# AFIDclan/cuda-raytracing

Hardware: AMD Instinct MI355X
Metric: Mrays/sec + ms/frame, 70k-tri OBJ at 1920x1080 1spp; 1/2/4/8 MI355X (higher is better)
Workload: dtype f32

## Files before the change

cuda-raytracing_amd/csrc/rt_device_types.h:

```cpp
#pragma once
#include <cstdint>
#include "rt_math.h"

namespace rt {

constexpr int32_t kLeafFlag = (int32_t)0x80000000u;
constexpr int kSlotBits = 26;
constexpr int32_t kSlotMask = (1 << kSlotBits) - 1;
constexpr int kMaxStack = 64;
constexpr int32_t kBoxUnordered = 1;

RT_HD bool boxes_ordered(const float* w)
{
    return w[0] <= w[3] && w[1] <= w[4] && w[2] <= w[5] && w[6] <= w[9] && w[7] <= w[10] && w[8] <= w[11];
}


struct DevInstance {
    Q4 q_rot;
    Q4 q_pose;
    Q4 q_inv_pose;
    Q4 q_inv_rot;
    float pose_xyz[3];
    float inv_pose_xyz[3];
    float scale[3];
    float inv_scale[3];
    int32_t root_ref;
    int32_t material_index;
    int32_t mesh_index;
    int32_t exact_uv;
    int32_t identity_inv;
    int32_t unit_inv;
    int32_t pad_[2];
};

struct DevMaterial {
    float albedo[3];
    int32_t texture_width;
    int32_t texture_height;
    uint32_t texture_pitch;
    const uint8_t* texture;
    float roughness, metallic;
};

constexpr int kExMaxGroup = 32;
constexpr int kExPlanesA = 5, kExPlanesS = 7;

constexpr int kMaxViewInstances = 8;
constexpr int kMaxBatch = 32;

struct FrameParams {
    float kinv[9];
    float D[4];
    float origin[3];
    Q4 q_cam;
    uint8_t* img;
    int32_t rank, local_rows;
};

struct RenderParams {
    int32_t width, height;
    int32_t num_frames;
    FrameParams frames[kMaxBatch];
    const float4* records;
    const float* tri_uv;
    const int32_t* tri_id;
    const int32_t* leaf_count;
    const int32_t* mesh_flags;
    const DevInstance* instances;
    const DevMaterial* materials;
    int32_t num_instances;
    int32_t stack_depth;
    uint64_t pitch;
    int32_t local_rows, stripe_rows, rank, num_ranks;
    int32_t tiles_x, tiles_y;
    unsigned long long* trace;
    const int32_t* tile_order;
    int32_t* tile_cost;
    int32_t spp, bounces, lighting;
    int32_t sample_base;
    float4* ex_samples;
// ... 29 lines not shown
```

cuda-raytracing_amd/csrc/rt_kernels.hip:

```cpp
#include <hip/hip_runtime.h>
#include <algorithm>
#include <cstddef>
#include <cstdio>
#include <cstdlib>
#include <cstring>
#include <mutex>
#include <new>
#include <type_traits>
#include <vector>

#include "../../include/rt_hip.h"
#include "rt_device_types.h"
#include "rt_math.h"
#include "rt_scene_internal.h"

using namespace rt;



namespace {

constexpr int kBlock = 256;
constexpr int kTile = 16;
constexpr int kPrimBlock = 64;
// ... 77 lines not shown
    lds_int* lds;
    int* spill;
    int lds_depth;
    int sp;
    __device__ __forceinline__ void push(int32_t v)
    {
        if constexpr (SPILL) { if (sp < lds_depth) lds[sp * STRIDE] = v; else spill[sp - lds_depth] = v; }
        else lds[sp * STRIDE] = v;
        sp++;
    }
    __device__ __forceinline__ int32_t pop()
    {
        --sp;
        if constexpr (!SPILL) return lds[sp * STRIDE];
        int32_t v = lds[(sp < lds_depth ? sp : lds_depth - 1) * STRIDE];
        if (sp >= lds_depth) v = spill[sp - lds_depth];
        return v;
    }
};

typedef StackT<kBlock> Stack;

struct MeshRay {
    V3 ro, rd, dinv;
};

__device__ __forceinline__ MeshRay to_mesh_space(const DevInstance& in, V3 org, V3 dir)
{
    MeshRay r;
    r.rd = apply_quat(in.q_rot, dir);
    r.rd.x *= in.inv_scale[0]; r.rd.y *= in.inv_scale[1]; r.rd.z *= in.inv_scale[2];
    r.ro = apply_quat(in.q_pose, v3(org.x - in.pose_xyz[0], org.y - in.pose_xyz[1], org.z - in.pose_xyz[2]));
    r.ro.x *= in.inv_scale[0]; r.ro.y *= in.inv_scale[1]; r.ro.z *= in.inv_scale[2];
    r.dinv = v3(1.0f / r.rd.x, 1.0f / r.rd.y, 1.0f / r.rd.z);
    return r;
}

template <bool DEBUG, class STK, int OCT = -1, bool NEED_POP = false, class W>
__device__ __forceinline__ bool interior_apply_words(const W& w, const MeshRay& r, float hit_min,
                                                     int32_t& cur, STK& stack, Counters<DEBUG>& cnt)
{
    int32_t ra = __float_as_int(w[12]), rb = __float_as_int(w[13]);
    if constexpr (DEBUG) cnt.aabb += 2;
    float da, db;
    if constexpr (OCT < 0) {
        da = slab(w[0], w[1], w[2], w[3], w[4], w[5], r.dinv);
        db = slab(w[6], w[7], w[8], w[9], w[10], w[11], r.dinv);
    } else {
        da = slab_oct<OCT>(w[0], w[1], w[2], w[3], w[4], w[5], r.dinv);
        db = slab_oct<OCT>(w[6], w[7], w[8], w[9], w[10], w[11], r.dinv);
    }
    const bool a_near = da < db;
    const bool pa = da < hit_min, pb = db < hit_min;
    int32_t next = pa ? ra : rb;
    if (pa && pb) {
        stack.push(a_near ? rb : ra);
        next = a_near ? ra : rb;
        if constexpr (STK::kOptimistic) next = stack.sp > stack.lds_depth ? kSentinel : next;
    }
    cur = NEED_POP ? ((pa | pb) ? next : kNeedPop) : next;
    return pa || pb;
}

template <bool DEBUG, class STK, int OCT = -1, bool NEED_POP = false>
__device__ __forceinline__ bool interior_apply(float4 q0, float4 q1, float4 q2, float4 q3, const MeshRay& r, float hit_min,
                                               int32_t& cur, STK& stack, Counters<DEBUG>& cnt)
// ... 23 lines not shown
    V3 pt = r.ro + tt * r.rd;
    ok = ok && !(pt.x == FLT_MAX);
    V3 e0 = v3(t1.z, t1.w, t2.x), e1 = v3(t2.y, t2.z, t2.w);
    V3 e2 = pt - v0;
    float dot02 = dot(e0, e2), dot12 = dot(e1, e2);
    float u = (t3.z * dot02 - t3.y * dot12) * t3.w;
    float v = (t3.x * dot12 - t3.y * dot02) * t3.w;
    ok = ok && (u >= 0.0f) && (v >= 0.0f) && (u + v <= 1.0f);
    c.u = u; c.v = v;
    if (exact_uv) {
        c.uv = make_float2(0.0f, 0.0f);
        if (ok) {
            const float* q = p.tri_uv + (size_t)slot * 6;
            float w = 1.0f - u - v;
            c.uv.x = (w * q[0] + v * q[2]) + u * q[4];
            c.uv.y = (w * q[1] + v * q[3]) + u * q[5];
            ok = c.uv.x != FLT_MAX;
        }
    }
    bool accept = false;
    if (ok) {
        if constexpr (DEBUG) cnt.inside++;
        V3 loc = pt;
        if (EX || !identity_inv) {
            loc = v3(pt.x * in.scale[0], pt.y * in.scale[1], pt.z * in.scale[2]);
            loc = apply_quat(in.q_inv_pose, v3(loc.x - in.inv_pose_xyz[0], loc.y - in.inv_pose_xyz[1], loc.z - in.inv_pose_xyz[2]));
        }
        c.dist = magnitude(loc - org);
        if constexpr (EX) c.loc = loc;
        accept = (denom < 0) & ((hit_min == FLT_MAX) | (c.dist < hit_min));
    }
    return accept;
}

template <bool DEBUG, bool PROF, bool EX, bool COUNT, class STK, bool POPS, int OCT, bool ANYHIT = false, bool VIEW = false>
__device__ __forceinline__ void trace_loop(const RenderParams& p, const DevInstance& in, int inst_index, const MeshRay& r,
                                           V3 org, STK& stack, Hit& hit, Counters<DEBUG>& cnt, int* iters, int* pops, uint32_t vdelta = 0,
                                           float tmax = FLT_MAX)
{
    static_assert(!VIEW || (!DEBUG && !PROF && !EX), "view records: the timed primary kernels only");
    stack.sp = 0;
    stack.push(kSentinel);
    int32_t cur = in.root_ref;
    bool have = true;
    constexpr bool kNeedPopValue = !EX;
    int rem = -1;
    unsigned long long c_pop = 0, c_mem = 0, c_int = 0, c_leaf = 0, n_it = 0, n_int = 0, n_leaf = 0, t0 = 0, t1 = 0, t2 = 0, t3 = 0;
    unsigned long long n_g1 = 0, n_g2 = 0, n_g34 = 0;
    const bool exact_uv = in.exact_uv != 0, identity_inv = in.identity_inv != 0;
    do {
        if constexpr (PROF) t1 = __builtin_amdgcn_s_memtime();
        if constexpr (COUNT) (*iters)++;
        const bool interior = cur >= 0;
        if constexpr (DEBUG) cnt.pops += (interior || rem < 0) ? 1 : 0;
        if constexpr (POPS) *pops += (interior || rem < 0) ? 1 : 0;
        float4 r0, r1, r2, r3;
        const int32_t cur0 = __builtin_amdgcn_readfirstlane(cur);
        typedef float f16v __attribute__((ext_vector_type(16)));
        if constexpr (VIEW) {
            const bool one_entry = __ballot(cur != cur0) == 0ull;
            if (one_entry && cur0 >= 0) {
                f16v w;
                const uint32_t off = ((uint32_t)cur0 << 6) + vdelta;
                asm volatile("s_load_dwordx16 %0, %1, %2\n\ts_waitcnt lgkmcnt(0)" : "=s"(w) : "s"(p.records), "s"(off));
                have = interior_apply_words<DEBUG, STK, OCT, kNeedPopValue>(w, r, hit.min, cur, stack, cnt);
                if (kNeedPopValue ? cur == kNeedPop : !have) cur = stack.pop();
// ... 79 lines not shown
        }
        if (any_accept != 0ull) {
            hit.min = accept ? c.dist : hit.min;
            hit.slot = accept ? slot : hit.slot;
            hit.instance = accept ? inst_index : hit.instance;
            hit.u = accept ? (exact_uv ? c.uv.x : c.u) : hit.u;
            hit.v = accept ? (exact_uv ? c.uv.y : c.v) : hit.v;
            if constexpr (EX) { hit.loc.x = accept ? c.loc.x : hit.loc.x; hit.loc.y = accept ? c.loc.y : hit.loc.y; hit.loc.z = accept ? c.loc.z : hit.loc.z; }
            if constexpr (ANYHIT) {
                const bool done = accept & (c.dist < tmax);
                if constexpr (kNeedPopValue) cur = done ? kSentinel : cur;
                else {
                    have = done ? false : have;
                    rem = done ? -1 : rem;
                    stack.sp = done ? 1 : stack.sp;
                }
            }
        }
        if constexpr (PROF) { __builtin_amdgcn_s_waitcnt(0); t0 = __builtin_amdgcn_s_memtime(); }
        if (kNeedPopValue ? cur == kNeedPop : !have) cur = stack.pop();
        __builtin_amdgcn_wave_barrier();
        if constexpr (PROF) {
            __builtin_amdgcn_s_waitcnt(0);
            c_mem += t2 - t1; c_int += t3 - t2; c_leaf += t0 - t3; c_pop += __builtin_amdgcn_s_memtime() - t0;
        }
    } while (cur != kSentinel);
    if constexpr (PROF) {
        if (p.trace) {
            unsigned long long v[10] = {c_pop, c_mem, c_int, c_leaf, n_it, n_int, n_leaf, n_g1, n_g2, n_g34};
            unsigned long long best = n_it;
            for (int o = 32; o > 0; o >>= 1) { unsigned long long x = __shfl_xor(best, o); best = x > best ? x : best; }
            const unsigned long long owner = __ballot(n_it == best);
            if ((int)(threadIdx.x & 63) == __ffsll((long long)owner) - 1) {
                unsigned long long* t = p.trace + (((size_t)blockIdx.y * gridDim.x + blockIdx.x) * (kPrimBlock / 64) + (threadIdx.x >> 6)) * 16 + 4;
                for (int k = 0; k < 10; k++) t[k] += v[k];
            }
        }
    }
}


#define RT_ASM_INTERIOR(AXN, AXF, AYN, AYF, AZN, AZF, BXN, BXF, BYN, BYF, BZN, BZF) \
    "v_mul_f32 v16, " AXN ", %[dix]\n\t"  "v_mul_f32 v17, " AYN ", %[diy]\n\t"  "v_mul_f32 v18, " AZN ", %[diz]\n\t" \
    "v_mul_f32 v19, " AXF ", %[dix]\n\t"  "v_mul_f32 v20, " AYF ", %[diy]\n\t"  "v_mul_f32 v21, " AZF ", %[diz]\n\t" \
    "v_max3_f32 v16, v16, v17, v18\n\t"                  \
    "v_min3_f32 v19, v19, v20, v21\n\t"                  \
    "v_mul_f32 v22, " BXN ", %[dix]\n\t"  "v_mul_f32 v23, " BYN ", %[diy]\n\t"  "v_mul_f32 v24, " BZN ", %[diz]\n\t" \
    "v_mul_f32 v25, " BXF ", %[dix]\n\t"  "v_mul_f32 v26, " BYF ", %[diy]\n\t"  "v_mul_f32 v27, " BZF ", %[diz]\n\t" \
    "v_max3_f32 v22, v22, v23, v24\n\t"                  \
    "v_min3_f32 v25, v25, v26, v27\n\t"                  \
    "v_cmp_ge_f32_e32 vcc, v19, v16\n\t" \
    "v_cmp_lt_f32_e64 s[38:39], 0, v19\n\t" \
    "v_cmp_lt_f32_e64 s[44:45], v16, %[hmin]\n\t" \
    "v_cmp_ge_f32_e64 s[40:41], v25, v22\n\t" \
    "v_cmp_lt_f32_e64 s[42:43], 0, v25\n\t" \
    "v_cmp_lt_f32_e64 s[66:67], v22, %[hmin]\n\t" \
    "v_cmp_lt_f32_e64 s[68:69], v16, v22\n\t"            \
    "s_and_b64 vcc, vcc, s[38:39]\n\t" \
    "s_and_b64 s[40:41], s[40:41], s[42:43]\n\t" \
    "s_and_b64 s[38:39], vcc, s[44:45]\n\t"              \
    "s_and_b64 s[40:41], s[40:41], s[66:67]\n\t"         \
    "s_orn2_b64 s[42:43], s[68:69], s[40:41]\n\t" \
    "s_and_b64 s[44:45], s[38:39], s[40:41]\n\t"         \
    "s_and_b64 s[42:43], s[42:43], s[38:39]\n\t"         \
    "s_or_b64 vcc, s[38:39], s[40:41]\n\t"               \
    "v_cndmask_b32_e64 v18, v13, v12, s[42:43]\n\t" \
    "s_and_saveexec_b64 s[38:39], s[44:45]\n\t" \
// ... 395 lines not shown
#undef RT_ASM_ORG_C
#undef RT_ASM_CASE_ANYHIT
    } else {
#define RT_ASM_ORG_C "s"
#define RT_ASM_CASE_ANYHIT(VN, SN)
        RT_ASM_ALL_CASES
#undef RT_ASM_ORG_C
#undef RT_ASM_CASE_ANYHIT
    }
#undef RT_ASM_ALL_CASES
#undef RT_ASM_CASE
#undef RT_ASM_VARIANT
#undef RT_ASM_ARGS
#undef RT_ASM_COUNT
#undef RT_ASM_NOCOUNT
#undef RT_ASM_GO
#undef RT_ASM_GO2
#undef RT_ASM_OUT_PLAIN
#undef RT_ASM_OUT_POPS
#undef RT_ASM_OUT_LOC
#undef RT_ASM_OUT_ANYHIT
#undef RT_ASM_STACK_OUT
#undef RT_ASM_STACK_IN
    sp = (int32_t)(sa - column) >> (ROW_SHIFT - 2);
}

__device__ __forceinline__ void loop_stat(const RenderParams& p, int which, unsigned long long n = 1ull)
{
    const unsigned long long active = __ballot(true);
    if ((int)(__lane_id()) == __ffsll((long long)active) - 1) atomicAdd(&p.loop_stats[which], n);
}

template <bool DEBUG, bool PROF, bool EX = false, bool COUNT = false, class STK = Stack, bool POPS = false, bool OCTANTS = true, bool ANYHIT = false,
          bool VIEW = false, bool UNIFORM_ORG = !EX, bool STATS = false, bool SEC = false>
__device__ __forceinline__ void trace_instance(const RenderParams& p, const DevInstance& in, int inst_index,
                                               V3 org, V3 dir, STK& stack, Hit& hit, Counters<DEBUG>& cnt, int* iters = nullptr,
                                               int* pops = nullptr, uint32_t view_off = 0, float tmax = FLT_MAX)
{
    const MeshRay r = to_mesh_space(in, org, dir);
    const uint32_t vdelta = VIEW ? view_off + (uint32_t)p.view_inst_off[inst_index] : 0u;
    int oct = -1;
    if constexpr (!PROF && OCTANTS) {
        const float inf = __int_as_float(0x7f800000);
        const bool usable = fabsf(r.dinv.x) < inf && fabsf(r.dinv.y) < inf && fabsf(r.dinv.z) < inf &&
                            r.dinv.x != 0.0f && r.dinv.y != 0.0f && r.dinv.z != 0.0f &&
                            fabsf(r.ro.x) < inf && fabsf(r.ro.y) < inf && fabsf(r.ro.z) < inf;
        const int mine = (r.dinv.x < 0.0f ? 1 : 0) | (r.dinv.y < 0.0f ? 2 : 0) | (r.dinv.z < 0.0f ? 4 : 0);
        const int first = __builtin_amdgcn_readfirstlane(mine);
        if ((p.mesh_flags[in.mesh_index] & 1) == 0 && __ballot(!usable || mine != first) == 0ull) oct = first;
    }
    static_assert(!SEC || (OCTANTS && POPS && !VIEW && !UNIFORM_ORG && !STK::kSpill && !DEBUG && !PROF && !COUNT), "SEC");
    if constexpr (SEC) { if (!(oct >= 0 && in.exact_uv == 0)) { stack.sp = 1; return; } }
    if constexpr (OCTANTS && !DEBUG && !PROF && (UNIFORM_ORG || SEC) && (!EX || POPS) && !(POPS && COUNT) && (!ANYHIT || SEC) && !STK::kSpill) {
        if (SEC || (oct >= 0 && in.exact_uv == 0)) {
            if constexpr (STATS) { loop_stat(p, RT_LOOP_ASM); if (in.unit_inv == 0) loop_stat(p, RT_LOOP_ASM_POSED); }
            stack.sp = 0;
            stack.push(kSentinel);
            int32_t cur = in.root_ref, sp = stack.sp;
            int wave_iters = 0;
            static_assert(STK::kStride == 64 || STK::kStride == 256, "the stack column's row pitch as a shift");
            int no_pops = 0;
            V3 point = v3(0.0f, 0.0f, 0.0f);
            const int32_t instance_before = hit.instance;
            if constexpr (EX) hit.instance = -7;
            const V3 back = v3(in.inv_pose_xyz[0], in.inv_pose_xyz[1], in.inv_pose_xyz[2]);
            const uintptr_t ia = in.unit_inv != 0 ? (uintptr_t)0 : (uintptr_t)&in;
            const DevInstance* general = (const DevInstance*)(((uintptr_t)(uint32_t)__builtin_amdgcn_readfirstlane((int)(uint32_t)(ia >> 32)) << 32) |
                                                              (uintptr_t)(uint32_t)__builtin_amdgcn_readfirstlane((int)(uint32_t)ia));
#define RT_TRACE_ASM(O) trace_loop_asm<O, COUNT, (STK::kStride == 64 ? 8 : 10), VIEW, POPS, EX, SEC, ANYHIT>(p, inst_index, r, org, stack.lds, stack.lds_depth, cur, sp, hit, wave_iters, vdelta, \
                                                                                              POPS ? *pops : no_pops, point, back, general, tmax)
            switch (oct) {
            case 0: RT_TRACE_ASM(0); break;
            case 1: RT_TRACE_ASM(1); break;
            case 2: RT_TRACE_ASM(2); break;
            case 3: RT_TRACE_ASM(3); break;
            case 4: RT_TRACE_ASM(4); break;
            case 5: RT_TRACE_ASM(5); break;
            case 6: RT_TRACE_ASM(6); break;
            default: RT_TRACE_ASM(7); break;
            }
#undef RT_TRACE_ASM
            stack.sp = sp;
            if constexpr (COUNT) *iters += wave_iters;
            if constexpr (EX) {
                if (hit.instance == -7) hit.instance = instance_before;
                else {
                    V3 loc = v3(point.x * in.scale[0], point.y * in.scale[1], point.z * in.scale[2]);
                    hit.loc = apply_quat(in.q_inv_pose, v3(loc.x - in.inv_pose_xyz[0], loc.y - in.inv_pose_xyz[1], loc.z - in.inv_pose_xyz[2]));
                }
            }
            return;
        }
    }
    if constexpr (SEC) return;
    else {
#define RT_TRACE_LOOP(O) trace_loop<DEBUG, PROF, EX, COUNT, STK, POPS, O, ANYHIT, (VIEW && !EX)>(p, in, inst_index, r, org, stack, hit, cnt, iters, pops, vdelta, tmax)
    if constexpr (STATS) loop_stat(p, STK::kSpill ? RT_LOOP_DEEP : (oct >= 0 ? RT_LOOP_CPP_OCTANT : RT_LOOP_CPP_GENERIC));
    switch (oct) {
    case 0: RT_TRACE_LOOP(0); break;
// ... 46 lines not shown

__device__ __forceinline__ void pixel_of(const RenderParams& p, const FrameParams& f, int tid, int x0, int y0, int& x, int& ly, int& y)
{
    const int wave = tid >> 6, lane = tid & 63;
    const int lx = lane & 7, lyy = lane >> 3;
    x = x0 + (wave & 1) * 8 + lx;
    ly = y0 + (wave >> 1) * 8 + lyy;
    y = ly;
    if (p.num_ranks != 1) y = ((ly / p.stripe_rows) * p.num_ranks + f.rank) * p.stripe_rows + ly % p.stripe_rows;
}

template <bool DEBUG, bool PROF, bool SPILL>
__host__ __device__ constexpr bool optimistic_stack() { return SPILL && !DEBUG && !PROF; }
template <bool DEBUG, bool PROF, bool SPILL>
__host__ __device__ inline int lds_block_rows(int stack_depth) { return lds_rows(stack_depth) + (optimistic_stack<DEBUG, PROF, SPILL>() ? 1 : 0); }

template <bool DEBUG, bool PROF, bool COUNT = false, bool SPILL = true, bool VIEW = false, bool STATS = false>
__device__ __forceinline__ void render_pixel(const RenderParams& p, const FrameParams& f, int x0, int y0, lds_int* lds_base, lds_int*& lds_column,
                                             int* iters = nullptr, uint32_t view_off = 0)
{
    int x, ly, y;
    pixel_of(p, f, (int)(lds_column - lds_base), x0, y0, x, ly, y);
    const V3 org = v3(f.origin[0], f.origin[1], f.origin[2]);
    const V3 dir = camera_direction(f, (float)x, (float)y);

    Hit hit;
    hit.min = FLT_MAX; hit.slot = -1; hit.instance = -1; hit.u = 0.0f; hit.v = 0.0f;
    Counters<DEBUG> cnt;
    if constexpr (optimistic_stack<DEBUG, PROF, SPILL>()) {
        StackT<kPrimBlock, false, true> stack;
        stack.lds = lds_column; stack.spill = nullptr; stack.lds_depth = lds_rows(p.stack_depth); stack.sp = 0;
        int outgrown = 0;
        for (int i = 0; i < p.num_instances; i++) {
            trace_instance<DEBUG, PROF, false, COUNT, StackT<kPrimBlock, false, true>, false, true, false, VIEW, true, STATS>(p, p.instances[i], i, org, dir, stack, hit, cnt,
                                                                                                                         iters, nullptr, view_off);
            outgrown |= stack.sp;
        }
        if constexpr (STATS) { loop_stat(p, RT_LOOP_WAVES); if (__ballot(outgrown != 0) != 0ull) loop_stat(p, RT_LOOP_RETRACED_LANES, (unsigned long long)__popcll(__ballot(outgrown != 0))); }
        if (outgrown != 0) {
            int spill[kMaxStack - kLdsStack];
            StackT<kPrimBlock, true> deep;
            deep.lds = lds_column; deep.spill = spill; deep.lds_depth = lds_rows(p.stack_depth); deep.sp = 0;
            hit.min = FLT_MAX; hit.slot = -1; hit.instance = -1; hit.u = 0.0f; hit.v = 0.0f;
            for (int i = 0; i < p.num_instances; i++)
                trace_instance<DEBUG, PROF, false, COUNT, StackT<kPrimBlock, true>, false, false, false, false, true, STATS>(p, p.instances[i], i, org, dir, deep, hit, cnt, iters);
        }
    } else {
        int spill[SPILL ? kMaxStack - kLdsStack : 1];
        StackT<kPrimBlock, SPILL> stack;
        stack.lds = lds_column; stack.spill = spill; stack.lds_depth = lds_rows(p.stack_depth); stack.sp = 0;
        if constexpr (STATS) loop_stat(p, RT_LOOP_WAVES);
        for (int i = 0; i < p.num_instances; i++)
            trace_instance<DEBUG, PROF, false, COUNT, StackT<kPrimBlock, SPILL>, false, true, false, VIEW, true, STATS>(p, p.instances[i], i, org, dir, stack, hit, cnt, iters,
                                                                                                               nullptr, view_off);
    }

    asm volatile("" : "+v"(lds_column));
    pixel_of(p, f, (int)(lds_column - lds_base), x0, y0, x, ly, y);
    const uint32_t px = shade(p, hit);
    uint8_t* out = f.img + (size_t)ly * p.pitch + 3 * (size_t)x;
    out[0] = (uint8_t)px; out[1] = (uint8_t)(px >> 8); out[2] = (uint8_t)(px >> 16);

    if (p.hit_instance || p.hit_triangle) {
        const size_t o = (size_t)y * p.width + x;
        if (p.hit_instance) p.hit_instance[o] = hit.instance;
        if (p.hit_triangle) p.hit_triangle[o] = hit.slot >= 0 ? p.tri_id[hit.slot] : -1;
    }
    if constexpr (DEBUG) {
        size_t o = (size_t)y * p.width + x;
        if (p.node_pops) p.node_pops[o] = cnt.pops;
        if (p.aabb_tests) p.aabb_tests[o] = cnt.aabb;
        if (p.tri_tests) p.tri_tests[o] = cnt.tris;
        if (p.inside_hits) p.inside_hits[o] = cnt.inside;
    }
}

template <bool DEBUG, bool PROF, bool ORDERED = false, bool SPILL = true, bool VIEW = false, bool STATS = false>
__global__ __launch_bounds__(kPrimBlock, 8) void render_kernel(const RenderParams p)
{
    extern __shared__ int lds_stack[];

    int tile = (int)blockIdx.x, frame = (int)blockIdx.y;
    int iters = 0;
    if constexpr (ORDERED) {
        frame = tile % p.num_frames;
        tile = tile / p.num_frames;
        if (p.tile_order) tile = p.tile_order[tile];
    }
    const int tx = tile % p.tiles_x, ty = tile / p.tiles_x;

    unsigned long long t_start = 0;
    if (p.trace) t_start = wall_clock64();
    lds_int* column = (lds_int*)lds_stack + threadIdx.x;
    {
        int x, ly, y;
        pixel_of(p, p.frames[frame], (int)threadIdx.x, tx * kPrimTile, ty * kPrimTile, x, ly, y);
        if (x < p.width && ly < p.frames[frame].local_rows)
            render_pixel<DEBUG, PROF, ORDERED, SPILL, VIEW, STATS>(p, p.frames[frame], tx * kPrimTile, ty * kPrimTile, (lds_int*)lds_stack, column, &iters,
                                                            VIEW ? p.view_base + (uint32_t)frame * p.view_frame_stride : 0u);
    }
    asm volatile("" : "+v"(column));
    const int tid = (int)(column - (lds_int*)lds_stack), wave = tid >> 6, lane = tid & 63;
    if constexpr (ORDERED) {
        static_assert(!ORDERED || kPrimBlock == 64, "one wave per workgroup: the wave's longest lane is the tile's");
        for (int o = 32; o > 0; o >>= 1) { const int v = __shfl_xor(iters, o); iters = v > iters ? v : iters; }
        if (p.tile_cost && lane < 9) {
            const int nx = tile % p.tiles_x + lane % 3 - 1, ny = tile / p.tiles_x + lane / 3 - 1;
            if (nx >= 0 && nx < p.tiles_x && ny >= 0 && ny < p.tiles_y) atomicMax(&p.tile_cost[ny * p.tiles_x + nx], iters);
        }
    }
    if (p.trace && lane == 0) {
        unsigned long long* t = p.trace + (((size_t)blockIdx.y * gridDim.x + blockIdx.x) * (kPrimBlock / 64) + wave) * 16;
        t[0] = t_start; t[1] = wall_clock64();
        unsigned hw; asm volatile("s_getreg_b32 %0, hwreg(HW_REG_HW_ID)" : "=s"(hw));
        unsigned xcc; asm volatile("s_getreg_b32 %0, hwreg(HW_REG_XCC_ID)" : "=s"(xcc));
        t[2] = ((unsigned long long)xcc << 32) | hw; t[3] = (unsigned long long)tile;
    }
}

__device__ __forceinline__ bool any_hit_done(const Hit& hit, float tmax)
{
    return hit.min < tmax && (tmax <= FLT_MAX || hit.instance >= 0);
}
template <bool LOC = true, bool OCTANTS = false, bool ANYHIT = false, class STK = Stack, bool OPTIMISTIC = false, bool VIEW = false, bool PRIMARY = false, bool SEC = false>
__device__ __forceinline__ Hit cast_ray_ex(const RenderParams& p, V3 org, V3 dir, STK& stack, int& pops, float tmax = FLT_MAX)
{
    static_assert(!VIEW || OPTIMISTIC, "view records are read by the LDS-only loops");
    static_assert(!SEC || (OCTANTS && OPTIMISTIC && !VIEW && !PRIMARY), "SEC");
    Hit hit;
    hit.min = FLT_MAX; hit.slot = -1; hit.instance = -1; hit.u = 0.0f; hit.v = 0.0f;
    hit.loc = v3(0.0f, 0.0f, 0.0f);
    Counters<false> none;
    if constexpr (OPTIMISTIC && STK::kSpill) {
        StackT<STK::kStride, false, true> fast;
        fast.lds = stack.lds; fast.spill = nullptr; fast.lds_depth = stack.lds_depth; fast.sp = 0;
        const int pops_before = pops;
        int outgrown = 0;
        for (int i = 0; i < p.num_instances; i++) {
            if constexpr (ANYHIT) { if (any_hit_done(hit, tmax)) continue; }
            trace_instance<false, false, LOC, false, StackT<STK::kStride, false, true>, true, OCTANTS, ANYHIT, VIEW, PRIMARY, false, SEC>(p, p.instances[i], i, org, dir, fast, hit, none,
                                                                                                                                        nullptr, &pops, p.view_base, tmax);
            outgrown |= (ANYHIT && SEC && any_hit_done(hit, tmax)) ? 0 : fast.sp;
        }
        if (outgrown == 0) return hit;
        pops = pops_before;
        hit.min = FLT_MAX; hit.slot = -1; hit.instance = -1; hit.u = 0.0f; hit.v = 0.0f;
        hit.loc = v3(0.0f, 0.0f, 0.0f);
    }
    for (int i = 0; i < p.num_instances; i++) {
// ... 577 lines not shown
    for (int l = 0; l < run.levels; l++) {
        for (int i = run.bound[l] + (int)threadIdx.x; i < run.bound[l + 1]; i += kRefitRunThreads) {
            float4* q = records + (size_t)sched[i] * 4;
            const float4 q3 = q[3];
            float amn[3], amx[3], bmn[3], bmx[3];
            refit_child_box(records, tri_id, leaf_count, vertices, __float_as_int(q3.x), amn, amx);
            refit_child_box(records, tri_id, leaf_count, vertices, __float_as_int(q3.y), bmn, bmx);
            q[0] = make_float4(amn[0], amn[1], amn[2], amx[0]);
            q[1] = make_float4(amx[1], amx[2], bmn[0], bmn[1]);
            q[2] = make_float4(bmn[2], bmx[0], bmx[1], bmx[2]);
            const float w[12] = {amn[0], amn[1], amn[2], amx[0], amx[1], amx[2], bmn[0], bmn[1], bmn[2], bmx[0], bmx[1], bmx[2]};
            if (!boxes_ordered(w)) *mesh_flag = kBoxUnordered;
        }
        __threadfence_block();
        __syncthreads();
    }
}

__global__ void set_instance_kernel(DevInstance* dst, const DevInstance value) { *dst = value; }

struct ViewJob {
    int32_t n;
    int32_t first[kMaxViewInstances];
    int32_t node_base[kMaxViewInstances];
    int32_t count[kMaxViewInstances];
    int32_t total;
};

__global__ __launch_bounds__(256) void view_records_kernel(const RenderParams p, const ViewJob job)
{
    const int t = (int)(blockIdx.x * 256 + threadIdx.x), frame = (int)blockIdx.y;
    int rec = t >> 2;
    const int quarter = t & 3;
    if (rec >= job.total) return;
    int i = 0;
    while (i + 1 < job.n && rec >= job.count[i]) { rec -= job.count[i]; i++; }
    const FrameParams& f = p.frames[frame];
    const V3 o = to_mesh_space(p.instances[i], v3(f.origin[0], f.origin[1], f.origin[2]), v3(0.0f, 0.0f, 1.0f)).ro;
    float4 v = p.records[(size_t)(job.node_base[i] + rec) * 4 + quarter];
    if (quarter == 0) v = make_float4(v.x - o.x, v.y - o.y, v.z - o.z, v.w - o.x);
    else if (quarter == 1) v = make_float4(v.x - o.y, v.y - o.z, v.z - o.x, v.w - o.y);
    else if (quarter == 2) v = make_float4(v.x - o.z, v.y - o.x, v.z - o.y, v.w - o.z);
    char* view = (char*)p.records + p.view_base + (size_t)frame * p.view_frame_stride;
    ((float4*)view)[(size_t)(job.first[i] + rec) * 4 + quarter] = v;
}

struct QueryParams {
    const float* org;
    const float* dir;
    const float* tmax;
    const int32_t* order;
    int32_t n;
    float* t;
    int32_t *instance, *triangle;
    float *location, *normal, *uv;
    int32_t* pops;
    uint8_t* occluded;
    int32_t* bins;
};
constexpr int kQueryBlock = 64;
typedef StackT<kQueryBlock> QueryStack;

__device__ __forceinline__ int32_t query_ray(const QueryParams& q, int32_t slot) { return q.order ? q.order[slot] : slot; }

template <bool ANYHIT>
__global__ __launch_bounds__(kQueryBlock, 8) void query_kernel(const RenderParams p, const QueryParams q)
{
    extern __shared__ int lds_stack[];
    const int32_t slot0 = (int32_t)blockIdx.x * kQueryBlock;
    if (slot0 + (int32_t)threadIdx.x >= q.n) return;
    int32_t i = query_ray(q, slot0 + (int32_t)threadIdx.x);
    const size_t i3 = (size_t)i * 3;
    const V3 org = v3(q.org[i3], q.org[i3 + 1], q.org[i3 + 2]);
    const V3 dir = v3(q.dir[i3], q.dir[i3 + 1], q.dir[i3 + 2]);
    const float tmax = (ANYHIT && q.tmax) ? q.tmax[i] : FLT_MAX;
    int spill[kMaxStack - kLdsStack];
// ... 2440 lines not shown
}

bool lds_stack_suffices(const RenderParams& p)
{
    static const bool forced = [] { const char* e = getenv("RT_STACK_SPILL"); return e && e[0] == '1'; }();
    return !forced && p.stack_depth - 1 <= kLdsStack;
}

constexpr size_t kViewMaxBytes = (size_t)3 << 30;

int view_mode()
{
    static const int mode = [] { const char* e = getenv("RT_VIEW_RECORDS"); return e && e[0] == '0' ? 0 : 1; }();
    return mode;
}

size_t view_budget()
{
    static const size_t b = [] {
        const char* e = getenv("RT_VIEW_MAX_BYTES");
        size_t v = e && *e ? (size_t)strtoull(e, nullptr, 10) : (size_t)1 << 30;
        return v > kViewMaxBytes ? kViewMaxBytes : v;
    }();
    return b;
}

void view_decide(RtScene* s)
{
    RtScene::ViewPool& v = s->view;
    if (v.decided) return;
    v.decided = true;
    int32_t cap = 0;
    for (const auto& rf : s->mesh_refit) cap = std::max(cap, rf.int_cap);
    v.frame_records = cap * (int32_t)s->instances.size();
    v.inst_first.resize(s->instances.size());
    for (size_t i = 0; i < s->instances.size(); i++) v.inst_first[i] = (int32_t)i * cap;
    v.usable = cap > 0 && s->records_bytes > 0 && !s->instances.empty() && s->instances.size() <= (size_t)kMaxViewInstances &&
               s->records_bytes + (size_t)v.frame_records * 64 <= kViewMaxBytes;
}

int view_resize(RtScene* s, int frames)
{
    RtScene::ViewPool& v = s->view;
    const size_t frame_bytes = (size_t)v.frame_records * 64, base = (s->records_bytes + 255) & ~(size_t)255;
    const size_t room = std::min(view_budget(), kViewMaxBytes > base ? kViewMaxBytes - base : 0);
    int slots = 3;
    while (slots > 1 && frame_bytes * (size_t)slots * (size_t)frames > room) slots--;
    if (frames < 1 || frame_bytes * (size_t)slots * (size_t)frames > room) return RT_E_NOMEM;
    const size_t total = base + frame_bytes * (size_t)slots * (size_t)frames;
    float4* block = nullptr;
    RT_HIP(hipDeviceSynchronize());
    if (hipMalloc((void**)&block, total) != hipSuccess) { (void)hipGetLastError(); return RT_E_NOMEM; }
    hipError_t e = hipMemcpy(block, s->d_records, s->records_bytes, hipMemcpyDeviceToDevice);
    if (e != hipSuccess) { (void)hipFree(block); return (int)e; }
    (void)hipFree(s->d_records);
    s->device_bytes += total;
    s->device_bytes -= std::min(s->device_bytes, s->records_alloc_bytes);
    s->d_records = block;
    s->records_alloc_bytes = total;
    v.base_bytes = base; v.slot_frames = frames; v.slots = slots; v.grows++;
    for (auto& sl : v.slot) { sl.used = false; sl.stream = nullptr; }
    return RT_OK;
}

int view_prepare(RtScene* s, RenderParams& p, hipStream_t stream, int samples = 1)
{
    if (!view_mode() || !s || p.num_instances < 1 || p.num_instances > kMaxViewInstances || p.num_ranks < 1) return -1;
    RtScene::ViewPool& v = s->view;
    view_decide(s);
// ... 12 lines not shown
                                             job.total, p.num_frames, min_frames, (long long)p.width * p.local_rows, min_rays);
        return -1;
    }
    auto count = [&](uint64_t RtScene::ViewPool::*field) { std::lock_guard<std::mutex> lock(v.m); (v.*field)++; };
    count(&RtScene::ViewPool::launches);
    const size_t frame_bytes = (size_t)v.frame_records * 64;
    if (p.num_frames > v.slot_frames) {
        if (v.reserved) { count(&RtScene::ViewPool::fallbacks); return -1; }
        int want = 1;
        while (want < p.num_frames) want = want == 1 ? 4 : want * 2;
        want = std::min(want, (int)kMaxBatch);
        int rc = view_resize(s, want);
        if (rc == RT_E_NOMEM && want != p.num_frames) rc = view_resize(s, p.num_frames);
        if (rc != RT_OK) {
            if (rc != RT_E_NOMEM) v.usable = false;
            count(&RtScene::ViewPool::fallbacks);
            return -1;
        }
    }
    int use = -1;
    for (int k = 0; k < v.slots && use < 0; k++) if (v.slot[k].used && v.slot[k].stream == stream) use = k;
    for (int k = 0; k < v.slots && use < 0; k++) if (!v.slot[k].used) use = k;
    for (int k = 0; k < v.slots && use < 0; k++) {
        if (hipEventQuery(v.slot[k].done) == hipSuccess) use = k;
        else (void)hipGetLastError();
    }
    if (use < 0) { count(&RtScene::ViewPool::fallbacks); return -1; }
    if (!v.slot[use].done && hipEventCreateWithFlags(&v.slot[use].done, hipEventDisableTiming) != hipSuccess) { count(&RtScene::ViewPool::fallbacks); return -1; }
    v.slot[use].used = true; v.slot[use].stream = stream;
    p.records = s->d_records;
    p.view_base = (uint32_t)(v.base_bytes + (size_t)use * v.slot_frames * frame_bytes);
    p.view_frame_stride = (uint32_t)frame_bytes;
    for (int i = 0; i < job.n; i++) p.view_inst_off[i] = (int32_t)(((int64_t)job.first[i] - job.node_base[i]) * 64);
    hipLaunchKernelGGL(view_records_kernel, dim3((unsigned)(((size_t)job.total * 4 + 255) / 256), (unsigned)p.num_frames), dim3(256), 0, stream, p, job);
    if (hipGetLastError() != hipSuccess) { count(&RtScene::ViewPool::fallbacks); return -1; }
    return use;
}

void view_done(RtScene* s, int slot, hipStream_t stream)
{
    if (slot < 0) return;
    (void)hipEventRecord(s->view.slot[slot].done, stream);
}

int launch_ordered(RtScene* s, RenderParams& p, hipStream_t stream, int synchronize, bool view)
{
    RtScene::TileOrderCache& cache = s->order;
    std::lock_guard<std::mutex> lock(cache.m);
    const int ntiles = p.tiles_x * p.tiles_y;
    if (!cache.sort_stream) RT_HIP(hipStreamCreateWithFlags(&cache.sort_stream, hipStreamNonBlocking));
    RtScene::TileOrder* o = nullptr;
    for (auto& e : cache.entry) if (e.ntiles && e.tiles_x == p.tiles_x && e.tiles_y == p.tiles_y) o = &e;
    if (!o) {
        for (auto& e : cache.entry) if (!e.ntiles && !o) o = &e;
        if (!o) {
            RtScene::TileOrder* lru = nullptr;
            for (auto& e : cache.entry) if (!lru || e.last_used < lru->last_used) lru = &e;
            if (order_state_idle(*lru)) {
                (void)hipFree(lru->d_cost);
                lru->d_cost = lru->d_keys = lru->d_order[0] = lru->d_order[1] = nullptr;
                lru->tiles_x = lru->tiles_y = lru->ntiles = 0; lru->cur = -1; lru->pending = false; lru->launches = lru->sorted_at = 0;
                for (auto& e : lru->seen) e.used = e.dirty = e.recorded = false;
                o = lru;
            }
        }
        if (o) {
            if (!o->sort_done) {
// ... 35 lines not shown
        }
        o->sorted_at = o->launches + 1;
        o->target = o->cur < 0 ? 0 : o->cur ^ 1;
        for (auto& e : o->seen) if (e.used && e.recorded) RT_HIP(hipStreamWaitEvent(cache.sort_stream, e.done, 0));
        hipLaunchKernelGGL(tile_sort_kernel, dim3(1), dim3(kSortThreads), 0, cache.sort_stream, o->d_cost, ntiles, o->d_keys, o->d_order[o->target]);
        RT_HIP(hipGetLastError());
        RT_HIP(hipEventRecord(o->sort_done, cache.sort_stream));
        o->pending = true;
    }
    const size_t lds = (size_t)(lds_stack_suffices(p) ? lds_block_rows<false, false, false>(p.stack_depth) : lds_block_rows<false, false, true>(p.stack_depth)) *
                       kPrimBlock * sizeof(int) + 2 * sizeof(int);
    const dim3 grid((unsigned)ntiles * (unsigned)p.num_frames);
    if (lds_stack_suffices(p)) {
        if (view) hipLaunchKernelGGL((render_kernel<false, false, true, false, true>), grid, dim3(kPrimBlock), lds, stream, p);
        else hipLaunchKernelGGL((render_kernel<false, false, true, false>), grid, dim3(kPrimBlock), lds, stream, p);
    } else {
        if (view) hipLaunchKernelGGL((render_kernel<false, false, true, true, true>), grid, dim3(kPrimBlock), lds, stream, p);
        else hipLaunchKernelGGL((render_kernel<false, false, true>), grid, dim3(kPrimBlock), lds, stream, p);
    }
    RT_HIP(hipGetLastError());
    if (o) o->launches++;
    if (mine) mine->dirty = true;
    if (synchronize) RT_HIP(hipStreamSynchronize(stream));
    return RT_OK;
}

int launch(RenderParams& p, bool debug, hipStream_t stream, int synchronize, RtScene* scene = nullptr, bool stats = false)
{
    if (p.width <= 0 || p.local_rows < 0) return RT_E_INVALID;
    if (p.local_rows == 0) return RT_OK;
    p.tiles_x = (p.width + kPrimTile - 1) / kPrimTile;
    p.tiles_y = (p.local_rows + kPrimTile - 1) / kPrimTile;
    const size_t lds = (size_t)(lds_stack_suffices(p) ? lds_rows(p.stack_depth) : lds_block_rows<false, false, true>(p.stack_depth)) * kPrimBlock * sizeof(int);
    dim3 grid((unsigned)(p.tiles_x * p.tiles_y), (unsigned)p.num_frames), block(kPrimBlock);
    const char* trace_file = getenv("RT_TRACE_FILE");
    const bool trace_ordered = trace_file && getenv("RT_TRACE_ORDERED");
    const int view_slot = (scene && !debug && !trace_file) ? view_prepare(scene, p, stream) : -1;
    struct ViewDone {
        RtScene* s; int slot; hipStream_t stream;
        ~ViewDone() { view_done(s, slot, stream); }
    } view_guard{scene, view_slot, stream};
    if (scene && !debug && (!trace_file || trace_ordered) && !p.hit_instance && !p.hit_triangle && grid.x >= 1024 && (size_t)grid.x * grid.y <= ((size_t)1 << 30)) {
        static const bool enabled = [] { const char* e = getenv("RT_TILE_ORDER"); return !(e && e[0] == '0'); }();
        static const bool stripes_too = [] { const char* e = getenv("RT_TILE_ORDER_STRIPES"); return !(e && e[0] == '0'); }();
        const bool thin_stripes = stripes_too && p.num_ranks > 1 && p.num_frames > 1 && (size_t)grid.x * grid.y < (size_t)4 * 32768;
        if (enabled && !stats && ((p.num_frames == 1 && grid.x >= 8192) || thin_stripes)) {
            if (!trace_ordered) return launch_ordered(scene, p, stream, synchronize, view_slot >= 0);
            const size_t n = (size_t)grid.x * (kPrimBlock / 64) * 16;
            RT_HIP(trace_begin(p, n));
            const int rc = launch_ordered(scene, p, stream, 1, false);
            const hipError_t e = trace_end(p, n, trace_file, stream);
            return rc ? rc : (int)e;
        }
    }
    const size_t trace_n = (size_t)grid.x * grid.y * (kPrimBlock / 64) * 16;
    if (trace_file) RT_HIP(trace_begin(p, trace_n));
    if (trace_file && getenv("RT_TRACE_PROF")) hipLaunchKernelGGL((render_kernel<false, true>), grid, block, lds, stream, p);
    else if (debug) hipLaunchKernelGGL((render_kernel<true, false>), grid, block, lds, stream, p);
    else if (stats) {
        if (lds_stack_suffices(p)) {
            if (view_slot >= 0) hipLaunchKernelGGL((render_kernel<false, false, false, false, true, true>), grid, block, lds, stream, p);
            else hipLaunchKernelGGL((render_kernel<false, false, false, false, false, true>), grid, block, lds, stream, p);
        } else {
            if (view_slot >= 0) hipLaunchKernelGGL((render_kernel<false, false, false, true, true, true>), grid, block, lds, stream, p);
            else hipLaunchKernelGGL((render_kernel<false, false, false, true, false, true>), grid, block, lds, stream, p);
        }
    }
    else if (lds_stack_suffices(p)) {
        if (view_slot >= 0) hipLaunchKernelGGL((render_kernel<false, false, false, false, true>), grid, block, lds, stream, p);
        else hipLaunchKernelGGL((render_kernel<false, false, false, false>), grid, block, lds, stream, p);
    } else {
        if (view_slot >= 0) hipLaunchKernelGGL((render_kernel<false, false, false, true, true>), grid, block, lds, stream, p);
        else hipLaunchKernelGGL((render_kernel<false, false>), grid, block, lds, stream, p);
    }
    RT_HIP(hipGetLastError());
    if (trace_file) RT_HIP(trace_end(p, trace_n, trace_file, stream));
    if (synchronize) RT_HIP(hipStreamSynchronize(stream));
    return RT_OK;
}

}

extern "C" {

int rt_abi_version(void) { return RT_ABI_VERSION; }

#ifndef RT_CODE_HASH
#define RT_CODE_HASH "built-without-it"
// ... 1652 lines not shown
```

Baseline: 20890.

## Precompute per-instance ray headers in view records and load via scalar fetch

The view-records kernel now also writes a 64-byte per-frame, per-instance header holding the mesh-space origin, rotation, inverse scale, root, flags and view offset. The primary trace path loads it with four s_load_dwordx4 instructions, which skips the per-lane origin transform, the mesh_flags lookup and several scattered DevInstance loads. The render grid also becomes 3D (tiles_x, tiles_y, frames), so tile coordinates no longer need a divide and modulo. The risks are that the inline-asm load waits on lgkmcnt(0), which forces a full scalar-memory wait, and that the view record region grows by one header per instance.

Result: faster. 21670 (median of 6 runs) (+3.7%).

```diff
diff --git a/cuda-raytracing_amd/csrc/rt_device_types.h b/cuda-raytracing_amd/csrc/rt_device_types.h
--- a/cuda-raytracing_amd/csrc/rt_device_types.h
+++ b/cuda-raytracing_amd/csrc/rt_device_types.h
@@ -47,6 +47,18 @@
 constexpr int kExPlanesA = 5, kExPlanesS = 7;
 
 constexpr int kMaxViewInstances = 8;
+struct RayHeader {
+    float ro[3];
+    uint32_t flags;
+    Q4 q_rot;
+    float inv_scale[3];
+    int32_t root_ref;
+    float inv_pose_xyz[3];
+    uint32_t vdelta;
+};
+static_assert(sizeof(RayHeader) == 64, "one scalar fetch of sixteen words");
+constexpr uint32_t kRayOriginFinite = 1, kRayBoxUnordered = 2, kRayExactUv = 4, kRayUnitInv = 8;
+
 constexpr int kMaxBatch = 32;
 
 struct FrameParams {
diff --git a/cuda-raytracing_amd/csrc/rt_kernels.hip b/cuda-raytracing_amd/csrc/rt_kernels.hip
--- a/cuda-raytracing_amd/csrc/rt_kernels.hip
+++ b/cuda-raytracing_amd/csrc/rt_kernels.hip
@@ -133,6 +133,38 @@
     r.rd.x *= in.inv_scale[0]; r.rd.y *= in.inv_scale[1]; r.rd.z *= in.inv_scale[2];
     r.ro = apply_quat(in.q_pose, v3(org.x - in.pose_xyz[0], org.y - in.pose_xyz[1], org.z - in.pose_xyz[2]));
     r.ro.x *= in.inv_scale[0]; r.ro.y *= in.inv_scale[1]; r.ro.z *= in.inv_scale[2];
+    r.dinv = v3(1.0f / r.rd.x, 1.0f / r.rd.y, 1.0f / r.rd.z);
+    return r;
+}
+
+struct RayHeaderWords {
+    V3 ro; uint32_t flags; Q4 q_rot; V3 inv_scale; int32_t root_ref; V3 back; uint32_t vdelta;
+};
+static_assert(offsetof(RayHeader, flags) == 12 && offsetof(RayHeader, q_rot) == 16 && offsetof(RayHeader, inv_scale) == 32 &&
+              offsetof(RayHeader, root_ref) == 44 && offsetof(RayHeader, inv_pose_xyz) == 48 && offsetof(RayHeader, vdelta) == 60, "RayHeader layout");
+
+__device__ __forceinline__ RayHeaderWords ray_header(const RenderParams& p, uint32_t view_off, int inst_index)
+{
+    typedef float f4v __attribute__((ext_vector_type(4)));
+    f4v w0, w1, w2, w3;
+    const uint32_t off = (uint32_t)__builtin_amdgcn_readfirstlane((int)(view_off + (uint32_t)inst_index * (uint32_t)sizeof(RayHeader)));
+    asm volatile("s_load_dwordx4 %0, %4, %5\n\ts_load_dwordx4 %1, %4, %5 offset:16\n\ts_load_dwordx4 %2, %4, %5 offset:32\n\t"
+                 "s_load_dwordx4 %3, %4, %5 offset:48\n\ts_waitcnt lgkmcnt(0)"
+                 : "=&s"(w0), "=&s"(w1), "=&s"(w2), "=&s"(w3) : "s"(p.records), "s"(off));
+    RayHeaderWords h;
+    h.ro = v3(w0[0], w0[1], w0[2]); h.flags = __float_as_uint(w0[3]);
+    h.q_rot.x = w1[0]; h.q_rot.y = w1[1]; h.q_rot.z = w1[2]; h.q_rot.w = w1[3];
+    h.inv_scale = v3(w2[0], w2[1], w2[2]); h.root_ref = __float_as_int(w2[3]);
+    h.back = v3(w3[0], w3[1], w3[2]); h.vdelta = __float_as_uint(w3[3]);
+    return h;
+}
+
+__device__ __forceinline__ MeshRay to_mesh_space(const RayHeaderWords& h, V3 dir)
+{
+    MeshRay r;
+    r.rd = apply_quat(h.q_rot, dir);
+    r.rd.x *= h.inv_scale.x; r.rd.y *= h.inv_scale.y; r.rd.z *= h.inv_scale.z;
+    r.ro = h.ro;
     r.dinv = v3(1.0f / r.rd.x, 1.0f / r.rd.y, 1.0f / r.rd.z);
     return r;
 }
@@ -222,6 +254,8 @@
     }
     return accept;
 }
+
+__device__ __forceinline__ size_t trace_workgroup() { return ((size_t)blockIdx.z * gridDim.y + blockIdx.y) * gridDim.x + blockIdx.x; }
 
 template <bool DEBUG, bool PROF, bool EX, bool COUNT, class STK, bool POPS, int OCT, bool ANYHIT = false, bool VIEW = false>
 __device__ __forceinline__ void trace_loop(const RenderParams& p, const DevInstance& in, int inst_index, const MeshRay& r,
@@ -367,7 +401,7 @@
             for (int o = 32; o > 0; o >>= 1) { unsigned long long x = __shfl_xor(best, o); best = x > best ? x : best; }
             const unsigned long long owner = __ballot(n_it == best);
             if ((int)(threadIdx.x & 63) == __ffsll((long long)owner) - 1) {
-                unsigned long long* t = p.trace + (((size_t)blockIdx.y * gridDim.x + blockIdx.x) * (kPrimBlock / 64) + (threadIdx.x >> 6)) * 16 + 4;
+                unsigned long long* t = p.trace + (trace_workgroup() * (kPrimBlock / 64) + (threadIdx.x >> 6)) * 16 + 4;
                 for (int k = 0; k < 10; k++) t[k] += v[k];
             }
         }
@@ -829,39 +863,42 @@
 }
 
 template <bool DEBUG, bool PROF, bool EX = false, bool COUNT = false, class STK = Stack, bool POPS = false, bool OCTANTS = true, bool ANYHIT = false,
-          bool VIEW = false, bool UNIFORM_ORG = !EX, bool STATS = false, bool SEC = false>
+          bool VIEW = false, bool UNIFORM_ORG = !EX, bool STATS = false, bool SEC = false, bool HDR = false>
 __device__ __forceinline__ void trace_instance(const RenderParams& p, const DevInstance& in, int inst_index,
                                                V3 org, V3 dir, STK& stack, Hit& hit, Counters<DEBUG>& cnt, int* iters = nullptr,
                                                int* pops = nullptr, uint32_t view_off = 0, float tmax = FLT_MAX)
 {
-    const MeshRay r = to_mesh_space(in, org, dir);
-    const uint32_t vdelta = VIEW ? view_off + (uint32_t)p.view_inst_off[inst_index] : 0u;
+    static_assert(!HDR || (VIEW && UNIFORM_ORG && OCTANTS && !EX && !SEC && !PROF && !DEBUG), "ray headers: the timed primary kernels' view path");
+    const RayHeaderWords h = HDR ? ray_header(p, view_off, inst_index) : RayHeaderWords();
+    const MeshRay r = HDR ? to_mesh_space(h, dir) : to_mesh_space(in, org, dir);
+    const uint32_t vdelta = HDR ? h.vdelta : VIEW ? view_off + (uint32_t)p.view_inst_off[inst_index] : 0u;
     int oct = -1;
     if constexpr (!PROF && OCTANTS) {
         const float inf = __int_as_float(0x7f800000);
         const bool usable = fabsf(r.dinv.x) < inf && fabsf(r.dinv.y) < inf && fabsf(r.dinv.z) < inf &&
                             r.dinv.x != 0.0f && r.dinv.y != 0.0f && r.dinv.z != 0.0f &&
-                            fabsf(r.ro.x) < inf && fabsf(r.ro.y) < inf && fabsf(r.ro.z) < inf;
+                            (HDR || (fabsf(r.ro.x) < inf && fabsf(r.ro.y) < inf && fabsf(r.ro.z) < inf));
         const int mine = (r.dinv.x < 0.0f ? 1 : 0) | (r.dinv.y < 0.0f ? 2 : 0) | (r.dinv.z < 0.0f ? 4 : 0);
         const int first = __builtin_amdgcn_readfirstlane(mine);
-        if ((p.mesh_flags[in.mesh_index] & 1) == 0 && __ballot(!usable || mine != first) == 0ull) oct = first;
+        if ((HDR ? (h.flags & (kRayOriginFinite | kRayBoxUnordered)) == kRayOriginFinite : (p.mesh_flags[in.mesh_index] & 1) == 0) &&
+            __ballot(!usable || mine != first) == 0ull) oct = first;
     }
     static_assert(!SEC || (OCTANTS && POPS && !VIEW && !UNIFORM_ORG && !STK::kSpill && !DEBUG && !PROF && !COUNT), "SEC");
     if constexpr (SEC) { if (!(oct >= 0 && in.exact_uv == 0)) { stack.sp = 1; return; } }
     if constexpr (OCTANTS && !DEBUG && !PROF && (UNIFORM_ORG || SEC) && (!EX || POPS) && !(POPS && COUNT) && (!ANYHIT || SEC) && !STK::kSpill) {
-        if (SEC || (oct >= 0 && in.exact_uv == 0)) {
-            if constexpr (STATS) { loop_stat(p, RT_LOOP_ASM); if (in.unit_inv == 0) loop_stat(p, RT_LOOP_ASM_POSED); }
+        if (SEC || (oct >= 0 && (HDR ? (h.flags & kRayExactUv) == 0 : in.exact_uv == 0))) {
+            if constexpr (STATS) { loop_stat(p, RT_LOOP_ASM); if (HDR ? (h.flags & kRayUnitInv) == 0 : in.unit_inv == 0) loop_stat(p, RT_LOOP_ASM_POSED); }
             stack.sp = 0;
             stack.push(kSentinel);
-            int32_t cur = in.root_ref, sp = stack.sp;
+            int32_t cur = HDR ? h.root_ref : in.root_ref, sp = stack.sp;
             int wave_iters = 0;
             static_assert(STK::kStride == 64 || STK::kStride == 256, "the stack column's row pitch as a shift");
             int no_pops = 0;
             V3 point = v3(0.0f, 0.0f, 0.0f);
             const int32_t instance_before = hit.instance;
             if constexpr (EX) hit.instance = -7;
-            const V3 back = v3(in.inv_pose_xyz[0], in.inv_pose_xyz[1], in.inv_pose_xyz[2]);
-            const uintptr_t ia = in.unit_inv != 0 ? (uintptr_t)0 : (uintptr_t)&in;
+            const V3 back = HDR ? h.back : v3(in.inv_pose_xyz[0], in.inv_pose_xyz[1], in.inv_pose_xyz[2]);
+            const uintptr_t ia = (HDR ? (h.flags & kRayUnitInv) != 0 : in.unit_inv != 0) ? (uintptr_t)0 : (uintptr_t)&in;
             const DevInstance* general = (const DevInstance*)(((uintptr_t)(uint32_t)__builtin_amdgcn_readfirstlane((int)(uint32_t)(ia >> 32)) << 32) |
                                                               (uintptr_t)(uint32_t)__builtin_amdgcn_readfirstlane((int)(uint32_t)ia));
 #define RT_TRACE_ASM(O) trace_loop_asm<O, COUNT, (STK::kStride == 64 ? 8 : 10), VIEW, POPS, EX, SEC, ANYHIT>(p, inst_index, r, org, stack.lds, stack.lds_depth, cur, sp, hit, wave_iters, vdelta, \
@@ -974,7 +1011,7 @@
         stack.lds = lds_column; stack.spill = nullptr; stack.lds_depth = lds_rows(p.stack_depth); stack.sp = 0;
         int outgrown = 0;
         for (int i = 0; i < p.num_instances; i++) {
-            trace_instance<DEBUG, PROF, false, COUNT, StackT<kPrimBlock, false, true>, false, true, false, VIEW, true, STATS>(p, p.instances[i], i, org, dir, stack, hit, cnt,
+            trace_instance<DEBUG, PROF, false, COUNT, StackT<kPrimBlock, false, true>, false, true, false, VIEW, true, STATS, false, VIEW>(p, p.instances[i], i, org, dir, stack, hit, cnt,
                                                                                                                          iters, nullptr, view_off);
             outgrown |= stack.sp;
         }
@@ -993,7 +1030,7 @@
         stack.lds = lds_column; stack.spill = spill; stack.lds_depth = lds_rows(p.stack_depth); stack.sp = 0;
         if constexpr (STATS) loop_stat(p, RT_LOOP_WAVES);
         for (int i = 0; i < p.num_instances; i++)
-            trace_instance<DEBUG, PROF, false, COUNT, StackT<kPrimBlock, SPILL>, false, true, false, VIEW, true, STATS>(p, p.instances[i], i, org, dir, stack, hit, cnt, iters,
+            trace_instance<DEBUG, PROF, false, COUNT, StackT<kPrimBlock, SPILL>, false, true, false, VIEW, true, STATS, false, VIEW>(p, p.instances[i], i, org, dir, stack, hit, cnt, iters,
                                                                                                                nullptr, view_off);
     }
 
@@ -1022,14 +1059,14 @@
 {
     extern __shared__ int lds_stack[];
 
-    int tile = (int)blockIdx.x, frame = (int)blockIdx.y;
+    int tile = (int)blockIdx.x, frame = ORDERED ? 0 : (int)blockIdx.z;
     int iters = 0;
     if constexpr (ORDERED) {
         frame = tile % p.num_frames;
         tile = tile / p.num_frames;
         if (p.tile_order) tile = p.tile_order[tile];
     }
-    const int tx = tile % p.tiles_x, ty = tile / p.tiles_x;
+    const int tx = ORDERED ? tile % p.tiles_x : (int)blockIdx.x, ty = ORDERED ? tile / p.tiles_x : (int)blockIdx.y;
 
     unsigned long long t_start = 0;
     if (p.trace) t_start = wall_clock64();
@@ -1052,11 +1089,12 @@
         }
     }
     if (p.trace && lane == 0) {
-        unsigned long long* t = p.trace + (((size_t)blockIdx.y * gridDim.x + blockIdx.x) * (kPrimBlock / 64) + wave) * 16;
+        const size_t wg = ORDERED ? (size_t)blockIdx.y * gridDim.x + blockIdx.x : trace_workgroup();
+        unsigned long long* t = p.trace + (wg * (kPrimBlock / 64) + wave) * 16;
         t[0] = t_start; t[1] = wall_clock64();
         unsigned hw; asm volatile("s_getreg_b32 %0, hwreg(HW_REG_HW_ID)" : "=s"(hw));
         unsigned xcc; asm volatile("s_getreg_b32 %0, hwreg(HW_REG_XCC_ID)" : "=s"(xcc));
-        t[2] = ((unsigned long long)xcc << 32) | hw; t[3] = (unsigned long long)tile;
+        t[2] = ((unsigned long long)xcc << 32) | hw; t[3] = (unsigned long long)(ORDERED ? tile : (int)(blockIdx.y * gridDim.x + blockIdx.x));
     }
 }
 
@@ -1700,16 +1738,32 @@
     const int t = (int)(blockIdx.x * 256 + threadIdx.x), frame = (int)blockIdx.y;
     int rec = t >> 2;
     const int quarter = t & 3;
-    if (rec >= job.total) return;
+    const FrameParams& f = p.frames[frame];
+    char* view = (char*)p.records + p.view_base + (size_t)frame * p.view_frame_stride;
+    if (rec >= job.total) {
+        const int i = t - job.total * 4;
+        if (i >= job.n) return;
+        const DevInstance& in = p.instances[i];
+        const V3 o = to_mesh_space(in, v3(f.origin[0], f.origin[1], f.origin[2]), v3(0.0f, 0.0f, 1.0f)).ro;
+        const float inf = __int_as_float(0x7f800000);
+        const uint32_t flags = (fabsf(o.x) < inf && fabsf(o.y) < inf && fabsf(o.z) < inf ? kRayOriginFinite : 0u) |
+                               ((p.mesh_flags[in.mesh_index] & kBoxUnordered) != 0 ? kRayBoxUnordered : 0u) |
+                               (in.exact_uv != 0 ? kRayExactUv : 0u) | (in.unit_inv != 0 ? kRayUnitInv : 0u);
+        const uint32_t vdelta = p.view_base + (uint32_t)frame * p.view_frame_stride + (uint32_t)p.view_inst_off[i];
+        float4* h = (float4*)view + (size_t)i * 4;
+        h[0] = make_float4(o.x, o.y, o.z, __uint_as_float(flags));
+        h[1] = make_float4(in.q_rot.x, in.q_rot.y, in.q_rot.z, in.q_rot.w);
+        h[2] = make_float4(in.inv_scale[0], in.inv_scale[1], in.inv_scale[2], __int_as_float(in.root_ref));
+        h[3] = make_float4(in.inv_pose_xyz[0], in.inv_pose_xyz[1], in.inv_pose_xyz[2], __uint_as_float(vdelta));
+        return;
+    }
     int i = 0;
     while (i + 1 < job.n && rec >= job.count[i]) { rec -= job.count[i]; i++; }
-    const FrameParams& f = p.frames[frame];
     const V3 o = to_mesh_space(p.instances[i], v3(f.origin[0], f.origin[1], f.origin[2]), v3(0.0f, 0.0f, 1.0f)).ro;
     float4 v = p.records[(size_t)(job.node_base[i] + rec) * 4 + quarter];
     if (quarter == 0) v = make_float4(v.x - o.x, v.y - o.y, v.z - o.z, v.w - o.x);
     else if (quarter == 1) v = make_float4(v.x - o.y, v.y - o.z, v.z - o.x, v.w - o.y);
     else if (quarter == 2) v = make_float4(v.x - o.z, v.y - o.x, v.z - o.y, v.w - o.z);
-    char* view = (char*)p.records + p.view_base + (size_t)frame * p.view_frame_stride;
     ((float4*)view)[(size_t)(job.first[i] + rec) * 4 + quarter] = v;
 }
 
@@ -4216,9 +4270,10 @@
     v.decided = true;
     int32_t cap = 0;
     for (const auto& rf : s->mesh_refit) cap = std::max(cap, rf.int_cap);
-    v.frame_records = cap * (int32_t)s->instances.size();
+    const int32_t headers = (int32_t)s->instances.size();
+    v.frame_records = headers + cap * (int32_t)s->instances.size();
     v.inst_first.resize(s->instances.size());
-    for (size_t i = 0; i < s->instances.size(); i++) v.inst_first[i] = (int32_t)i * cap;
+    for (size_t i = 0; i < s->instances.size(); i++) v.inst_first[i] = headers + (int32_t)i * cap;
     v.usable = cap > 0 && s->records_bytes > 0 && !s->instances.empty() && s->instances.size() <= (size_t)kMaxViewInstances &&
                s->records_bytes + (size_t)v.frame_records * 64 <= kViewMaxBytes;
 }
@@ -4297,7 +4352,7 @@
     p.view_base = (uint32_t)(v.base_bytes + (size_t)use * v.slot_frames * frame_bytes);
     p.view_frame_stride = (uint32_t)frame_bytes;
     for (int i = 0; i < job.n; i++) p.view_inst_off[i] = (int32_t)(((int64_t)job.first[i] - job.node_base[i]) * 64);
-    hipLaunchKernelGGL(view_records_kernel, dim3((unsigned)(((size_t)job.total * 4 + 255) / 256), (unsigned)p.num_frames), dim3(256), 0, stream, p, job);
+    hipLaunchKernelGGL(view_records_kernel, dim3((unsigned)(((size_t)job.total * 4 + (size_t)job.n + 255) / 256), (unsigned)p.num_frames), dim3(256), 0, stream, p, job);
     if (hipGetLastError() != hipSuccess) { count(&RtScene::ViewPool::fallbacks); return -1; }
     return use;
 }
@@ -4399,7 +4454,8 @@
     p.tiles_x = (p.width + kPrimTile - 1) / kPrimTile;
     p.tiles_y = (p.local_rows + kPrimTile - 1) / kPrimTile;
     const size_t lds = (size_t)(lds_stack_suffices(p) ? lds_rows(p.stack_depth) : lds_block_rows<false, false, true>(p.stack_depth)) * kPrimBlock * sizeof(int);
-    dim3 grid((unsigned)(p.tiles_x * p.tiles_y), (unsigned)p.num_frames), block(kPrimBlock);
+    const size_t ntiles = (size_t)p.tiles_x * p.tiles_y, nframes = (size_t)p.num_frames;
+    dim3 grid((unsigned)p.tiles_x, (unsigned)p.tiles_y, (unsigned)p.num_frames), block(kPrimBlock);
     const char* trace_file = getenv("RT_TRACE_FILE");
     const bool trace_ordered = trace_file && getenv("RT_TRACE_ORDERED");
     const int view_slot = (scene && !debug && !trace_file) ? view_prepare(scene, p, stream) : -1;
@@ -4407,20 +4463,21 @@
         RtScene* s; int slot; hipStream_t stream;
         ~ViewDone() { view_done(s, slot, stream); }
     } view_guard{scene, view_slot, stream};
-    if (scene && !debug && (!trace_file || trace_ordered) && !p.hit_instance && !p.hit_triangle && grid.x >= 1024 && (size_t)grid.x * grid.y <= ((size_t)1 << 30)) {
+    if (scene && !debug && (!trace_file || trace_ordered) && !p.hit_instance && !p.hit_triangle && ntiles >= 1024 && ntiles * nframes <= ((size_t)1 << 30)) {
         static const bool enabled = [] { const char* e = getenv("RT_TILE_ORDER"); return !(e && e[0] == '0'); }();
         static const bool stripes_too = [] { const char* e = getenv("RT_TILE_ORDER_STRIPES"); return !(e && e[0] == '0'); }();
-        const bool thin_stripes = stripes_too && p.num_ranks > 1 && p.num_frames > 1 && (size_t)grid.x * grid.y < (size_t)4 * 32768;
-        if (enabled && !stats && ((p.num_frames == 1 && grid.x >= 8192) || thin_stripes)) {
+        const bool thin_stripes = stripes_too && p.num_ranks > 1 && p.num_frames > 1 && ntiles * nframes < (size_t)4 * 32768;
+        if (enabled && !stats && ((p.num_frames == 1 && ntiles >= 8192) || thin_stripes)) {
             if (!trace_ordered) return launch_ordered(scene, p, stream, synchronize, view_slot >= 0);
-            const size_t n = (size_t)grid.x * (kPrimBlock / 64) * 16;
+            const size_t n = ntiles * nframes * (kPrimBlock / 64) * 16;
             RT_HIP(trace_begin(p, n));
             const int rc = launch_ordered(scene, p, stream, 1, false);
             const hipError_t e = trace_end(p, n, trace_file, stream);
             return rc ? rc : (int)e;
         }
     }
-    const size_t trace_n = (size_t)grid.x * grid.y * (kPrimBlock / 64) * 16;
+    if (p.tiles_y > 65535) return RT_E_INVALID;
+    const size_t trace_n = ntiles * nframes * (kPrimBlock / 64) * 16;
     if (trace_file) RT_HIP(trace_begin(p, trace_n));
     if (trace_file && getenv("RT_TRACE_PROF")) hipLaunchKernelGGL((render_kernel<false, true>), grid, block, lds, stream, p);
     else if (debug) hipLaunchKernelGGL((render_kernel<true, false>), grid, block, lds, stream, p);
```
